# Critical-Infrastructure-Systems-Lab/ldsr

Hardware: AMD Instinct MI355X
Metric: restart x EM-iteration / s (T=1000, p=1, q=2) (higher is better)
Workload: dtype f64; 1 GPU; cfg2: synthetic T=1000 p=1 q=2, 1 series x 4096 restarts/GPU, niter=100, tol=0, dense mask; cells_rank0=4096, cells_total=4096, niter=100, algo=3

## Files before the change

### ldsr_amd/csrc/em_pair_impl.h

```cpp
#pragma once
#include "em_scan_impl.h"

__host__ __device__ constexpr long pair_image_doubles(int L, int PP, int QQ, int LPC = 32) {
    return img_doubles(L, LPC, PP, QQ);
}
__host__ __device__ constexpr long pair_strip_doubles(int L) { return (long)64 * (L - 1); }

__host__ __device__ constexpr long pair_tri_doubles(int PP, int QQ, int LPC = 32) {
    return (long)LPC * 2 * scan_pairs(PP, QQ);
}
#ifndef LDSR_STEADY
#define LDSR_STEADY 1
#endif
#ifndef LDSR_STEADY_PF
#define LDSR_STEADY_PF 4
#endif
#ifndef LDSR_STEADY_PF2
#define LDSR_STEADY_PF2 6
#endif
#ifndef LDSR_LEAD_CLOSED_VAR
#define LDSR_LEAD_CLOSED_VAR 1
#endif
#ifndef LDSR_STEADY_SBMASK
#define LDSR_STEADY_SBMASK 0x6
// ... 537 lines not shown
                    for (int p_ = 0; p_ < PP; p_++) bu = fma(th.B[p_], un[p_], bu);
                    if constexpr (LPF) {
                        const int jn = min(j + 1, nj - 1);
#pragma unroll
                        for (int p_ = 0; p_ < PP; p_++) un[p_] = lup[(long)jn * LPC * PP + p_];
                    }
                    bl = fma(A, bl, bu);
                    if constexpr (!LDSR_LEAD_CLOSED_VAR) {
                        ql = fma(A2, ql, Q);
                        al *= A;
                        a2l *= A2;
                    }
                }
            }
            if constexpr (LDSR_LEAD_CLOSED_VAR) {
                double pa = A, pa2 = A2;
#pragma unroll
                for (int bit = 0; bit < 10; bit++) {
                    if ((nj >> bit) & 1) { al *= pa; a2l *= pa2; }
                    pa *= pa; pa2 *= pa2;
                }
                const double omA2 = 1.0 - A2;
                var_closed = fabs(omA2) > 0.0009765625;
                if (var_closed) {
                    const double romA2 = fast_rcp(omA2);
                    geo = (1.0 - a2l) * romA2;
                    ql = Q * geo;
                    geo2 = ((double)nj - geo) * romA2;
                } else {
                    for (int j = 0; j < nj; j++) ql = fma(A2, ql, Q);
                }
            }
#define LSCAN_ROUND(AB, BB, A2B, QB)                                       \
            {                                                              \
                const double ab = AB, bb = BB, a2b = A2B, qb = QB;         \
                bl = fma(al, bb, bl);  al *= ab;                           \
                ql = fma(a2l, qb, ql); a2l *= a2b;                         \
            }
            LSCAN_ROUND(dpp1<DPP_ROW_SHR(1)>(al), dppz<DPP_ROW_SHR(1)>(bl), dpp1<DPP_ROW_SHR(1)>(a2l), dppz<DPP_ROW_SHR(1)>(ql))
            LSCAN_ROUND(dpp1<DPP_ROW_SHR(2)>(al), dppz<DPP_ROW_SHR(2)>(bl), dpp1<DPP_ROW_SHR(2)>(a2l), dppz<DPP_ROW_SHR(2)>(ql))
            LSCAN_ROUND(dpp1<DPP_ROW_SHR(4)>(al), dppz<DPP_ROW_SHR(4)>(bl), dpp1<DPP_ROW_SHR(4)>(a2l), dppz<DPP_ROW_SHR(4)>(ql))
            LSCAN_ROUND(dpp1<DPP_ROW_SHR(8)>(al), dppz<DPP_ROW_SHR(8)>(bl), dpp1<DPP_ROW_SHR(8)>(a2l), dppz<DPP_ROW_SHR(8)>(ql))
            if constexpr (LPC == 32)
                LSCAN_ROUND((dppd<DPP_ROW_BCAST15, 0xA>(1.0, al)), (dppd<DPP_ROW_BCAST15, 0xA>(0.0, bl)),
                            (dppd<DPP_ROW_BCAST15, 0xA>(1.0, a2l)), (dppd<DPP_ROW_BCAST15, 0xA>(0.0, ql)))
#undef LSCAN_ROUND
            double Xl = fma(al, th.mu1, bl), Vl = fma(a2l, th.V1, ql);
            x_t1 = shfl_d(Xl, hbase | (LPC - 1));
            v_t1 = shfl_d(Vl, hbase | (LPC - 1));
            Xl = dppd<DPP_WAVE_SHR1, 0xF>(th.mu1, Xl);
            Vl = dppd<DPP_WAVE_SHR1, 0xF>(th.V1, Vl);
            if (vl == 0) { Xl = th.mu1; Vl = th.V1; }
            const double rV1 = fast_rcp(v_t1);
            const double As = fabs(A) < 1e-150 ? copysign(1e-150, A) : A;
            const double rA = fast_rcp(As);
            const int k0 = lead - tA;
            const double xl2 = (double)k0 * (log_pos(fabs(As)) * 1.4426950408889634074);
            const double ef = fmin(fmax(floor(xl2), -1.0e6), 1.0e6);
            double dm = exp2(xl2 - ef);
            int de = (int)ef;
            if (As < 0.0 && (k0 & 1)) dm = -dm;
            dm *= rV1;
            de += __builtin_amdgcn_frexp_exp(dm);
            dm = __builtin_amdgcn_frexp_mant(dm);
            c_first = __builtin_amdgcn_ldexp(dm, de) * Vl;
            c_first = shfl_d(c_first, hbase);
            l_X = Xl; l_V = Vl; l_dm = dm; l_de = de; l_rA = rA; l_nj = nj;
            l_closed = var_closed; l_geo = geo; l_geo2 = geo2;
        }

        double likq = 0.0, lsp = 0.0, tLv = 0.0, X0v = 0.0, V0v = 0.0;
        int sneg = 0;
        double aSyx, aTx1x, aPall, aSxx = 0.0;
        double aSxv[QQ], aTx1u[PP], aTux[PP];
        auto zero_sums = [&]() {
            aSyx = 0.0; aTx1x = 0.0; aPall = 0.0;
#pragma unroll
            for (int q_ = 0; q_ < QQ; q_++) aSxv[q_] = 0.0;
#pragma unroll
            for (int p_ = 0; p_ < PP; p_++) { aTx1u[p_] = 0.0; aTux[p_] = 0.0; }
        };

        SCAN_TICK(0)
        if (alive) {
            PairSweepOut<PP, QQ> o;
            pair_generic_sweeps<PP, QQ, L, LPC, DENSE>(o, th, ys, hs, obsmask, lane, nl, rp, x_t1, v_t1);
            aSyx = o.aSyx; aTx1x = o.aTx1x; aPall = o.aPall; aSxx = o.aSxx;
            likq = o.likq; lsp = o.lsp; tLv = o.tLv; X0v = o.X0v; V0v = o.V0v; sneg = o.sneg;
#pragma unroll
            for (int q_ = 0; q_ < QQ; q_++) aSxv[q_] = o.aSxv[q_];
#pragma unroll
            for (int p_ = 0; p_ < PP; p_++) { aTx1u[p_] = o.aTx1u[p_]; aTux[p_] = o.aTux[p_]; }
        } else {
            zero_sums();
        }

        SCAN_TICK(6)
        if constexpr (LEAD) {
            const double dlt = shfl_d(X0v, hbase) - x_t1;
            const double *lup = lu + (long)vl * PP;
            constexpr bool LPF = LPC == 32;
            const int nj = l_nj;
            const double rA = l_rA;
            double Xl = l_X, Vl = l_V, dm = l_dm;
            int de = l_de;
#pragma unroll
            for (int i = 0; i < NLS; i++) lS[i] = 0.0;
            double c = __builtin_amdgcn_ldexp(dm, de) * Vl;
            double Xs = fma(c, dlt, Xl);
            auto lead2 = [&](int j, const double (&ul)[PP]) {
                double bu = 0.0;
#pragma unroll
                for (int p_ = 0; p_ < PP; p_++) bu = fma(th.B[p_], ul[p_], bu);
                const double Xl1 = fma(A, Xl, bu), Vl1 = fma(A2, Vl, Q);
                dm *= rA;
                if ((j & 3) == 3) { de += __builtin_amdgcn_frexp_exp(dm); dm = __builtin_amdgcn_frexp_mant(dm); }
                const double c1 = __builtin_amdgcn_ldexp(dm, de) * Vl1;
                const double Xs1 = fma(c1, dlt, Xl1);
                lS[0] = fma(Xs, Xs, lS[0]);
                if constexpr (!LDSR_LEAD_CLOSED_VAR) lS[1] += Vl;
                lS[2] = fma(c, c, lS[2]);
                lS[3] = fma(Xs1, Xs, lS[3]);
                lS[4] = fma(c, c1, lS[4]);
#pragma unroll
                for (int p_ = 0; p_ < PP; p_++) {
                    lS[5 + p_] = fma(Xs1, ul[p_], lS[5 + p_]);
                    lS[5 + PP + p_] = fma(ul[p_], Xs, lS[5 + PP + p_]);
                }
                Xl = Xl1; Vl = Vl1; c = c1; Xs = Xs1;
            };
            if constexpr (lead_pipe(PP)) {
                const int nA = (lead + LPC - 1) / LPC;
                lead_walk<PP, LPC>(lup, nj, nA, lead2);
            } else {
                double un2[PP];
#pragma unroll
                for (int p_ = 0; p_ < PP; p_++) un2[p_] = (LPF && nj > 0) ? lup[p_] : 0.0;
                for (int j = 0; j < nj; j++) {
                    double ul[PP];
                    if constexpr (!LPF) {
#pragma unroll
                        for (int p_ = 0; p_ < PP; p_++) un2[p_] = lup[(long)j * LPC * PP + p_];
                    }
#pragma unroll
                    for (int p_ = 0; p_ < PP; p_++) ul[p_] = un2[p_];
                    if constexpr (LPF) {
                        const int jn = min(j + 1, nj - 1);
#pragma unroll
                        for (int p_ = 0; p_ < PP; p_++) un2[p_] = lup[(long)jn * LPC * PP + p_];
                    }
                    lead2(j, ul);
                }
            }
            if constexpr (LDSR_LEAD_CLOSED_VAR) {
                if (l_closed) {
                    lS[1] = fma(l_V, l_geo, Q * l_geo2);
                } else {
                    double vv = l_V;
                    for (int j = 0; j < nj; j++) { lS[1] += vv; vv = fma(A2, vv, Q); }
                }
            }
        }
        SCAN_TICK(5)
        Sums<PP, QQ> S;
        {
            constexpr int NB = 5 + (DENSE ? 0 : 1);
            constexpr int NT = NB + QQ + 2 * PP;
            constexpr int NR = NT + (LEAD ? NLS : 0);
            constexpr int NSL = (NR + LPC - 1) / LPC;
            static_assert(NSL <= 4, "reduction gather: at most four slots per lane");
            double red[NR];
            if constexpr (LEAD) {
#pragma unroll
                for (int i = 0; i < NLS; i++) red[NT + i] = lS[i];
            }
            red[0] = aSyx; red[1] = aTx1x; red[2] = aPall; red[3] = likq; red[4] = lsp;
            if (!DENSE) red[5] = aSxx;
#pragma unroll
            for (int q_ = 0; q_ < QQ; q_++) red[NB + q_] = aSxv[q_];
#pragma unroll
            for (int p_ = 0; p_ < PP; p_++) { red[NB + QQ + p_] = aTx1u[p_]; red[NB + QQ + PP + p_] = aTux[p_]; }
            red_rounds<NR, LPC / 2>(red, lane);
            {
                double tt[NSL];
#pragma unroll
                for (int k_ = 0; k_ < NSL; k_++) tt[k_] = red[k_];
#pragma unroll
                for (int i = 0; i < NR; i++) red[i] = shfl_d(tt[red_slot(i, NR, LPC)], hbase | red_home(i, NR, LPC));
            }
            S.X0 = shfl_d(X0v, hbase);
            S.V0 = shfl_d(V0v, hbase);
            const double termLast = shfl_d(tLv, hbase | lastLane);
            if constexpr (LEAD) {
                const double dlt = S.X0 - x_t1, eps = S.V0 - v_t1;
                const double *l = red + NT;
                red[2] += (l[0] + l[1]) + eps * l[2];
                red[1] += l[3] + fma(eps, l[4], A * l[1]);
#pragma unroll
                for (int p_ = 0; p_ < PP; p_++) {
                    red[NB + QQ + p_] += l[5 + p_];
                    red[NB + QQ + PP + p_] += l[5 + PP + p_];
                }
                S.X0 = fma(c_first, dlt, th.mu1);
                S.V0 = fma(c_first * c_first, eps, th.V1);
            }
            const double term0 = fma(S.X0, S.X0, S.V0);
            const unsigned long long negm = __ballot(sneg < 0);
            const bool neg = ((negm >> hbase) & ((1ull << LPC) - 1ull)) != 0;
            S.Syx = red[0]; S.Tx1x = red[1];
            S.Sxx = DENSE ? red[2] : red[5];
#pragma unroll
            for (int q_ = 0; q_ < QQ; q_++) S.Sxv[q_] = red[NB + q_];
#pragma unroll
            for (int p_ = 0; p_ < PP; p_++) { S.Tx1u[p_] = red[NB + QQ + p_]; S.Tux[p_] = red[NB + QQ + PP + p_]; }
            S.Txx = red[2] - termLast;
            S.Tx1x1 = red[2] - term0;
            lik2 = lik1;
            lik1 = lik;
            lik = (-0.5 * n_obs * LDSR_LOG_2PI - 0.5 * (red[3] + red[4])) / n_obs;
            if (neg) lik = NAN;
        }
        SCAN_TICK(8)
        int abort_now = 0;
        if (prm.abort && ((++wit) & 63) == 0)
            abort_now = __builtin_amdgcn_readfirstlane(lane == 0 ? ldsr_poll_abort(prm.abort) : 0);
        if (alive && prm.liks && vl == 0) prm.liks[(long)cell * prm.niter + it] = lik;
        it++;
        bool stop = it >= prm.niter || abort_now;
        if (it >= 3 && fabs(lik - lik1) < prm.tol && fabs(lik1 - lik2) < prm.tol) stop = true;
        if (alive && stop) {
            white_out(th, (SeriesConstK)sc);
            if (vl == 0) {
                store_theta(th, prm.theta + (long)cell * P, prm.p, prm.q);
                if (prm.liks && prm.liks_nanfill)
                    for (int i = it; i < prm.niter; i++) prm.liks[(long)cell * prm.niter + i] = NAN;
                prm.n_iter[cell] = it;
                prm.lik[cell] = lik;
                prm.status[cell] = (abort_now && it < prm.niter) ? 3 : (isfinite(lik) ? 0 : 1);
#ifdef LDSR_SCAN_TIMING
                tick_[9] = __builtin_amdgcn_s_memrealtime() - real0_;
                if (prm.liks && prm.niter >= 10)
                    for (int k_ = 0; k_ < 10; k_++) prm.liks[(long)cell * prm.niter + k_] = (double)tick_[k_];
#endif
            }
            alive = false;
            if constexpr (QUEUE) {
                if (abort_now) {
                    for (int pulls = 0; pulls <= nc; pulls++) {
                        int kn = 0;
                        if (vl == 0) kn = atomicAdd(prm.queue + s, 1);
                        kn = __shfl(kn, hbase, 64);
                        if (kn >= nc) break;
                        if (vl == 0) mark_cell_interrupted(prm, c0 + kn);
                    }
                }
                if (!abort_now) {
                    int kn = 0;
                    if (vl == 0) kn = atomicAdd(prm.queue + s, 1);
                    kn = __shfl(kn, hbase, 64);
                    if (kn < nc) {
                        alive = true;
                        cell = c0 + kn;
                        load_theta(th, prm.theta0 + (long)cell * P, prm.p, prm.q, prm.has_u, prm.has_v);
                        white_in(th, (SeriesConstK)sc);
                        it = 0;
                        lik = NAN; lik1 = NAN; lik2 = NAN;
                    }
                }
            }
        } else {
            mstep_update_white<PP, QQ>(th, S, (SeriesConstK)sc, T);
        }
    }
}


struct PairEnv {
    int T, p, q, has_u, has_v, niter, liks_nanfill, n_obs;
    double tol;
    const SeriesConst *sc;
    int *queue_s;
    const int *perm;
    const double *theta0;
    double *theta, *lik, *liks;
    int *n_iter, *status;
    const int *abort;
};
template <int PP, int QQ>
struct PairCarry {
    Theta<PP, QQ> th;
    double lik, lik1, lik2;
    int it, cell, wit;
    bool alive;
#ifdef LDSR_SCAN_TIMING
    unsigned long long tick_[10], last_, real0_;
#endif
};
#ifdef LDSR_SCAN_TIMING
#define PAIR_TICK_REFS auto &tick_ = cs.tick_; auto &last_ = cs.last_;
#else
#define PAIR_TICK_REFS
#endif

__device__ __forceinline__ int pair_cell_at(const PairEnv &E, int c0, int pos) { return E.perm ? E.perm[c0 + pos] : c0 + pos; }

__device__ __forceinline__ void pair_mark_interrupted(const PairEnv &E, int cell) {
    const int P = 6 + E.p + E.q;
    for (int k = 0; k < P; k++) E.theta[(long)cell * P + k] = NAN;
    if (E.liks && E.liks_nanfill)
        for (int i = 0; i < E.niter; i++) E.liks[(long)cell * E.niter + i] = NAN;
    E.n_iter[cell] = 0;
    E.lik[cell] = NAN;
    E.status[cell] = 3;
}

struct PairVarBlk { double Vp, sg, r0, K, Vu, AVu, J, Vp1; bool st; };
template <int L>
__device__ __forceinline__ PairVarBlk pair_var_block(double V1, double A, double C, double Q, double R, bool live,
                                                     int vl, int hbase, bool shape_ok) {
    constexpr int LPC = 32, NTR = L - 1;
    PairVarBlk b;
    const double A2 = A * A, C2 = C * C;
    const double C2R = C2 * fast_rcp(R), alpha = fma(Q, C2R, A2);
    const bool trl = vl < NTR;
    double Vp;
    {
        const double mxs = fmax(alpha, 1.0);
        const int ke = -__builtin_amdgcn_frexp_exp(mxs);
        const double cs = __builtin_amdgcn_ldexp(1.0, ke);
        double p00 = trl ? alpha * cs : 1.0, p01 = trl ? Q * cs : 0.0;
        double p10 = trl ? C2R * cs : 0.0, p11 = trl ? cs : 1.0;
#define VSCAN_ROUND(Q00, Q01, Q10, Q11)                                                      \
        {                                                                            \
            const double q00 = Q00, q01 = Q01, q10 = Q10, q11 = Q11;                 \
            const double r00 = fma(p00, q00, p01 * q10), r01 = fma(p00, q01, p01 * q11); \
            const double r10 = fma(p10, q00, p11 * q10), r11 = fma(p10, q01, p11 * q11); \
            p00 = r00; p01 = r01; p10 = r10; p11 = r11;                              \
        }
#define VSCAN_SHR(n) VSCAN_ROUND(dpp1<DPP_ROW_SHR(n)>(p00), dppz<DPP_ROW_SHR(n)>(p01), dppz<DPP_ROW_SHR(n)>(p10), dpp1<DPP_ROW_SHR(n)>(p11))
        VSCAN_SHR(1) VSCAN_SHR(2) VSCAN_SHR(4)
        {
            const double m = fmax(fmax(fabs(p00), fabs(p01)), fmax(fabs(p10), fabs(p11)));
            const int e2 = 1 - __builtin_amdgcn_frexp_exp(m);
            p00 = __builtin_amdgcn_ldexp(p00, e2); p01 = __builtin_amdgcn_ldexp(p01, e2);
            p10 = __builtin_amdgcn_ldexp(p10, e2); p11 = __builtin_amdgcn_ldexp(p11, e2);
        }
        VSCAN_SHR(8)
        VSCAN_ROUND((dppd<DPP_ROW_BCAST15, 0xA>(1.0, p00)), (dppd<DPP_ROW_BCAST15, 0xA>(0.0, p01)),
                    (dppd<DPP_ROW_BCAST15, 0xA>(0.0, p10)), (dppd<DPP_ROW_BCAST15, 0xA>(1.0, p11)))
#undef VSCAN_SHR
#undef VSCAN_ROUND
        double n_e = fma(p00, V1, p01), d_e = fma(p10, V1, p11);
        n_e = dppd<DPP_WAVE_SHR1, 0xF>(V1, n_e);
        d_e = dppd<DPP_WAVE_SHR1, 0xF>(1.0, d_e);
        if (vl == 0) { n_e = V1; d_e = 1.0; }
        Vp = n_e * fast_rcp(d_e);
    }
    const double sg = fma(C2, Vp, R);
    const double r0 = fast_rcp(sg);
    const double w = Vp * r0;
    b.K = C * w;
    b.Vu = R * w;
    b.Vp1 = fma(A2, b.Vu, Q);
    b.AVu = A * b.Vu;
    b.J = b.AVu * fast_rcp(b.Vp1);
    b.Vp = Vp; b.sg = sg; b.r0 = r0;
    const double dV = b.Vp1 - Vp;
    const bool conv = fabs(dV) <= 3.552713678800501e-15 * fabs(Vp) && Vp > 0.0 && b.J * b.J < 0.8;
    const unsigned long long okm = __ballot(sg > 0.0 && sg < INFINITY);
    const unsigned long long cvm = __ballot(conv);
    constexpr unsigned long long CELL = (1ull << LPC) - 1ull;
    const unsigned long long hm = (okm >> hbase) & CELL, hc = (cvm >> hbase) & CELL;
    b.st = live && hm == CELL && ((hc >> (LPC - 1)) & 1ull) != 0ull && shape_ok;
    return b;
}

template <int PP, int QQ, bool QUEUE>
__device__ __forceinline__ void pair_steady_finish(const PairEnv &E, PairCarry<PP, QQ> &cs, const PairSweepOut<PP, QQ> &o,
                                                   double addTx1x, double addPall, bool active, int lane, int c0,
                                                   int nc, int lastLane) {
    constexpr int LPC = 32;
    PAIR_TICK_REFS
    const int vl = lane & 31, hbase = lane & 32;
    const int P = 6 + E.p + E.q;
    Sums<PP, QQ> S;
    {
        constexpr int NB = 5;
        constexpr int NR = NB + QQ + 2 * PP;
        double red[NR];
        red[0] = o.aSyx; red[1] = o.aTx1x; red[2] = o.aPall; red[3] = o.likq; red[4] = o.lsp;
#pragma unroll
        for (int q_ = 0; q_ < QQ; q_++) red[NB + q_] = o.aSxv[q_];
#pragma unroll
        for (int p_ = 0; p_ < PP; p_++) { red[NB + QQ + p_] = o.aTx1u[p_]; red[NB + QQ + PP + p_] = o.aTux[p_]; }
        red_rounds<NR, LPC / 2>(red, lane);
        {
            const double tt = red[0];
#pragma unroll
            for (int i = 0; i < NR; i++) red[i] = shfl_d(tt, hbase | red_home(i, NR, LPC));
        }
        S.X0 = shfl_d(o.X0v, hbase);
        S.V0 = shfl_d(o.V0v, hbase);
        const double termLast = shfl_d(o.tLv, hbase | lastLane);
        red[1] += addTx1x; red[2] += addPall;
        const double term0 = fma(S.X0, S.X0, S.V0);
        const unsigned long long negm = __ballot(o.sneg < 0);
        const bool neg = ((negm >> hbase) & ((1ull << LPC) - 1ull)) != 0;
        S.Syx = red[0]; S.Tx1x = red[1];
        S.Sxx = red[2];
#pragma unroll
        for (int q_ = 0; q_ < QQ; q_++) S.Sxv[q_] = red[NB + q_];
#pragma unroll
        for (int p_ = 0; p_ < PP; p_++) { S.Tx1u[p_] = red[NB + QQ + p_]; S.Tux[p_] = red[NB + QQ + PP + p_]; }
        S.Txx = red[2] - termLast;
        S.Tx1x1 = red[2] - term0;
        if (active) {
            cs.lik2 = cs.lik1;
            cs.lik1 = cs.lik;
            cs.lik = (-0.5 * E.n_obs * LDSR_LOG_2PI - 0.5 * (red[3] + red[4])) / E.n_obs;
            if (neg) cs.lik = NAN;
        }
    }
    SCAN_TICK(8)
    int abort_now = 0;
    if (E.abort && ((++cs.wit) & 63) == 0)
        abort_now = __builtin_amdgcn_readfirstlane(lane == 0 ? ldsr_poll_abort(E.abort) : 0);
    if (active && E.liks && vl == 0) E.liks[(long)cs.cell * E.niter + cs.it] = cs.lik;
    if (active) cs.it++;
    bool stop = active && cs.it >= E.niter;
    if (active && cs.it >= 3 && fabs(cs.lik - cs.lik1) < E.tol && fabs(cs.lik1 - cs.lik2) < E.tol) stop = true;
    if (cs.alive && abort_now) stop = true;
    if (cs.alive && stop) {
        white_out(cs.th, (SeriesConstK)E.sc);
        if (vl == 0) {
            store_theta(cs.th, E.theta + (long)cs.cell * P, E.p, E.q);
            if (E.liks && E.liks_nanfill)
                for (int i = cs.it; i < E.niter; i++) E.liks[(long)cs.cell * E.niter + i] = NAN;
            E.n_iter[cs.cell] = cs.it;
            E.lik[cs.cell] = cs.lik;
            E.status[cs.cell] = (abort_now && cs.it < E.niter) ? 3 : (isfinite(cs.lik) ? 0 : 1);
#ifdef LDSR_SCAN_TIMING
            tick_[9] = __builtin_amdgcn_s_memrealtime() - cs.real0_;
            if (E.liks && E.niter >= 10)
                for (int k_ = 0; k_ < 10; k_++) E.liks[(long)cs.cell * E.niter + k_] = (double)tick_[k_];
#endif
        }
        cs.alive = false;
        if constexpr (QUEUE) {
            if (abort_now) {
                for (int pulls = 0; pulls <= nc; pulls++) {
                    int kn = 0;
                    if (vl == 0) kn = atomicAdd(E.queue_s, 1);
                    kn = __shfl(kn, hbase, 64);
                    if (kn >= nc) break;
                    if (vl == 0) pair_mark_interrupted(E, pair_cell_at(E, c0, kn));
                }
            } else {
                int kn = 0;
                if (vl == 0) kn = atomicAdd(E.queue_s, 1);
                kn = __shfl(kn, hbase, 64);
                if (kn < nc) {
                    cs.alive = true;
                    cs.cell = pair_cell_at(E, c0, kn);
                    load_theta(cs.th, E.theta0 + (long)cs.cell * P, E.p, E.q, E.has_u, E.has_v);
                    white_in(cs.th, (SeriesConstK)E.sc);
                    cs.it = 0;
                    cs.lik = NAN; cs.lik1 = NAN; cs.lik2 = NAN;
                }
            }
        }
    } else if (active) {
        mstep_update_white<PP, QQ>(cs.th, S, (SeriesConstK)E.sc, E.T);
    }
}

template <int PP, int QQ, int L, bool QUEUE>
__device__ __attribute__((noinline)) PairCarry<PP, QQ> pair_steady_g_phase(PairEnv Ev, PairCarry<PP, QQ> cs, bool slow,
                                                                           int c0, int nc) {
    constexpr int LPC = 32;
    extern __shared__ __attribute__((aligned(16))) double smem[];
    PAIR_TICK_REFS
    auto ui = [](int x) { return __builtin_amdgcn_readfirstlane(x); };
    auto up = [&](auto *ptr) {
        const unsigned long long v = (unsigned long long)ptr;
        const unsigned lo = (unsigned)__builtin_amdgcn_readfirstlane((int)(unsigned)v);
        const unsigned hi = (unsigned)__builtin_amdgcn_readfirstlane((int)(unsigned)(v >> 32));
        return (decltype(ptr))(((unsigned long long)hi << 32) | lo);
    };
    PairEnv E;
    E.T = ui(Ev.T); E.p = ui(Ev.p); E.q = ui(Ev.q); E.has_u = ui(Ev.has_u); E.has_v = ui(Ev.has_v);
    E.niter = ui(Ev.niter); E.liks_nanfill = ui(Ev.liks_nanfill); E.n_obs = ui(Ev.n_obs);
    E.tol = uniform_d(Ev.tol);
    E.sc = up(Ev.sc); E.queue_s = up(Ev.queue_s); E.perm = up(Ev.perm); E.theta0 = up(Ev.theta0);
    E.theta = up(Ev.theta); E.lik = up(Ev.lik); E.liks = up(Ev.liks); E.n_iter = up(Ev.n_iter);
    E.status = up(Ev.status); E.abort = up(Ev.abort);
    c0 = ui(c0); nc = ui(nc);
    const int lane = threadIdx.x & 63, wave = threadIdx.x >> 6;
    const int vl = lane & 31, hbase = lane & 32;
    const int T = E.T;
    const int nl = (T + L - 1) / L, rp = T - nl * (L - 1);
    const bool shape_ok = rp >= 1 && nl > 1;
    const double *ys = smem;
    double *hs = smem + pair_image_doubles(L, PP, QQ, LPC) + (long)wave * pair_strip_doubles(L) + lane;
    do {
        SCAN_TICK(7)
        PairSweepOut<PP, QQ> o;
        pair_generic_sweeps<PP, QQ, L, LPC, true>(o, cs.th, ys, hs, 0u, lane, nl, rp, cs.th.mu1, cs.th.V1);
        SCAN_TICK(6)
        pair_steady_finish<PP, QQ, QUEUE>(E, cs, o, 0.0, 0.0, slow, lane, c0, nc, nl - 1);
        const PairVarBlk vb = pair_var_block<L>(cs.th.V1, cs.th.A, cs.th.C, cs.th.Q, cs.th.R, cs.alive, vl, hbase, shape_ok);
        slow = cs.alive && !vb.st;
    } while (__any(slow));
    return cs;
}

template <int PP, int QQ, int L, bool QUEUE>
__device__ __forceinline__ void em_pair_body_steady(const EmParams &prm, const double *ys, double *hs,
                                                    const double *tri, int s, int c0, int nc, int lane,
                                                    int wave) {
    constexpr int LPC = 32;
    constexpr int KP = scan_pairs(PP, QQ), KV = img_values(PP, QQ);
    constexpr int NTR = L - 1;
    static_assert(NTR < LPC, "the last lane of the cell is the template, not a transient step");
    const int vl = lane & 31, hbase = lane & 32;
    auto val = [&](int j, int i) -> double { return ys[img_off(j, i, KV, LPC, L) + vl * 2]; };
    auto ldw = [&](int j, double (&w)[2 * KP]) {
#pragma unroll
        for (int i = 0; i < KV; i++) w[i] = val(j, i);
    };
    constexpr int PF = KP <= 2 ? LDSR_STEADY_PF : (KP <= 4 ? 2 : 1);
    constexpr int PF2 = LDSR_STEADY_PF2;
    const int T = prm.T;
    const int P = 6 + prm.p + prm.q;
    PairEnv E;
    E.T = T; E.p = prm.p; E.q = prm.q; E.has_u = prm.has_u; E.has_v = prm.has_v;
    E.niter = prm.niter; E.liks_nanfill = prm.liks_nanfill; E.tol = prm.tol;
    E.sc = prm.sc + s; E.n_obs = E.sc->n_obs;
    E.queue_s = prm.queue + s; E.perm = prm.perm; E.theta0 = prm.theta0;
    E.theta = prm.theta; E.lik = prm.lik; E.liks = prm.liks; E.n_iter = prm.n_iter; E.status = prm.status;
    E.abort = prm.abort;
    const int nl = (T + L - 1) / L;
    const int rp = T - nl * (L - 1);
    const bool act = vl < nl;
    const bool tail = vl < rp;
    const int lastLane = nl - 1;
    const bool shape_ok = rp >= 1 && nl > 1;

    PairCarry<PP, QQ> cs;
    int k = QUEUE ? 0 : 2 * wave + (lane >> 5);
    if constexpr (QUEUE) {
        if (vl == 0) k = atomicAdd(E.queue_s, 1);
        k = __shfl(k, hbase, 64);
    }
    cs.alive = k < nc;
    cs.cell = pair_cell_at(E, c0, cs.alive ? k : 0);
    load_theta(cs.th, prm.theta0 + (long)cs.cell * P, prm.p, prm.q, prm.has_u, prm.has_v);
    white_in(cs.th, (SeriesConstK)E.sc);
    cs.lik = NAN; cs.lik1 = NAN; cs.lik2 = NAN;
    cs.it = 0;
    cs.wit = 0;
#ifdef LDSR_SCAN_TIMING
    for (int k_ = 0; k_ < 10; k_++) cs.tick_[k_] = 0;
    cs.last_ = __builtin_readcyclecounter();
    cs.real0_ = __builtin_amdgcn_s_memrealtime();
#endif
    PAIR_TICK_REFS
    Theta<PP, QQ> &th = cs.th;

    while (__any(cs.alive)) {
        bool slow = false;
        while (__any(cs.alive)) {
            SCAN_TICK(7)
            const double A = th.A, C = th.C;
            const PairVarBlk vb = pair_var_block<L>(th.V1, A, C, th.Q, th.R, cs.alive, vl, hbase, shape_ok);
            const bool st = vb.st;
            slow = cs.alive && !st;
            if (__builtin_expect(__any(slow), 0)) break;
            double likq = 0.0, lsp = 0.0, tLv = 0.0, X0v = 0.0, V0v = 0.0;
            double addPall = 0.0, addTx1x = 0.0;
            double aSyx = 0.0, aTx1x = 0.0, aPall = 0.0;
            double aSxv[QQ], aTx1u[PP], aTux[PP];
            auto zero_sums = [&]() {
                aSyx = 0.0; aTx1x = 0.0; aPall = 0.0;
#pragma unroll
                for (int q_ = 0; q_ < QQ; q_++) aSxv[q_] = 0.0;
#pragma unroll
                for (int p_ = 0; p_ < PP; p_++) { aTx1u[p_] = 0.0; aTux[p_] = 0.0; }
            };
            const bool trl = vl < NTR;
            auto tval = [&](int i) -> double { return tri[((i >> 1) * LPC + vl) * 2 + (i & 1)]; };
            double e_t = tval(0), bu_t = 0.0;
#pragma unroll
            for (int q_ = 0; q_ < QQ; q_++) e_t = fma(-th.D[q_], tval(1 + PP + q_), e_t);
#pragma unroll
            for (int p_ = 0; p_ < PP; p_++) bu_t = fma(th.B[p_], tval(1 + p_), bu_t);
            const double K = vb.K, J = vb.J, Vu = vb.Vu, AVu = vb.AVu, r0 = vb.r0;
            double Xp;
            {
                const double aKt = A * K;
                double al = trl ? fma(-aKt, C, A) : 1.0, bl = trl ? fma(aKt, e_t, bu_t) : 0.0;
#define MSCAN_ROUND(AB, BB) { const double ab = AB, bb = BB; bl = fma(al, bb, bl); al *= ab; }
                MSCAN_ROUND(dpp1<DPP_ROW_SHR(1)>(al), dppz<DPP_ROW_SHR(1)>(bl))
                MSCAN_ROUND(dpp1<DPP_ROW_SHR(2)>(al), dppz<DPP_ROW_SHR(2)>(bl))
                MSCAN_ROUND(dpp1<DPP_ROW_SHR(4)>(al), dppz<DPP_ROW_SHR(4)>(bl))
                MSCAN_ROUND(dpp1<DPP_ROW_SHR(8)>(al), dppz<DPP_ROW_SHR(8)>(bl))
                MSCAN_ROUND((dppd<DPP_ROW_BCAST15, 0xA>(1.0, al)), (dppd<DPP_ROW_BCAST15, 0xA>(0.0, bl)))
#undef MSCAN_ROUND
                Xp = fma(al, th.mu1, bl);
                Xp = dppd<DPP_WAVE_SHR1, 0xF>(th.mu1, Xp);
                if (vl == 0) Xp = th.mu1;
            }
            const double dl = fma(-C, Xp, e_t);
            const double Xu = fma(K, dl, Xp);
            const double Xp1 = fma(A, Xu, bu_t);
            const double trJ = J;
            const double trG = fma(-J, Xp1, Xu);
            const double trH = fma(-J, AVu, Vu);
            const double trLq = trl ? dl * r0 * dl : 0.0;
            const double lg = log_pos(vb.sg);
            const double trLg = trl ? lg : 0.0;
            const int src = hbase | (LPC - 1);
            const double cK = shfl_d(K, src), cJ = shfl_d(J, src), cr = shfl_d(r0, src), cVu = shfl_d(Vu, src);
            const double ch = shfl_d(trH, src), clg = shfl_d(lg, src), X_tr = shfl_d(Xp, src);

            SCAN_TICK(0)
            if (st) {
                const bool body = act && vl >= 1;
                const bool tail_s = tail;
                const double aK = A * cK, a = fma(-aK, C, A);
                double aL = 1.0, JL = 1.0;
                {
                    double sa = a, sj = cJ;
                    bool have = false;
#pragma unroll
                    for (int bit = 0; (1 << bit) <= L - 1; bit++) {
                        if ((L - 1) & (1 << bit)) {
                            if (!have) { aL = sa; JL = sj; have = true; }
                            else { aL *= sa; JL *= sj; }
                        }
                        if ((2 << bit) <= L - 1) { sa *= sa; sj *= sj; }
                    }
                }
                double gv_[L];
                double al = 1.0, bl = 0.0, buLast = 0.0;
                auto f1s = [&](int j, const double (&w)[2 * KP]) {
                    double e = w[0], bu = 0.0;
#pragma unroll
                    for (int q_ = 0; q_ < QQ; q_++) e = fma(-th.D[q_], w[1 + PP + q_], e);
#pragma unroll
                    for (int p_ = 0; p_ < PP; p_++) bu = fma(th.B[p_], w[1 + p_], bu);
                    gv_[j] = e;
                    if (j < L - 1) hs[j * 64] = bu; else buLast = bu;
                    bl = fma(a, bl, fma(aK, e, bu));
                };
                {
                    constexpr bool PRET = KP <= 4;
                    double Wt[2 * KP], W[PF][2 * KP];
                    if constexpr (PRET) ldw(L - 1, Wt);
#pragma unroll
                    for (int d = 0; d < PF; d++) ldw(d, W[d]);
                    __builtin_amdgcn_sched_barrier(LDSR_STEADY_SBMASK);
                    if (body) {
#pragma unroll
                        for (int j = 0; j < L - 1; j++) {
                            f1s(j, W[j % PF]);
                            if (j + PF < L - 1) ldw(j + PF, W[j % PF]);
                            __builtin_amdgcn_sched_barrier(LDSR_STEADY_SBMASK);
                        }
                        al = aL;
                    }
                    if (tail_s) {
                        if constexpr (!PRET) ldw(L - 1, Wt);
                        f1s(L - 1, Wt);
                        al *= a;
                    }
                }
#define SSCAN_ROUND(AB, BB) { const double ab = AB, bb = BB; bl = fma(al, bb, bl); al *= ab; }
                SSCAN_ROUND(dpp1<DPP_ROW_SHR(1)>(al), dppz<DPP_ROW_SHR(1)>(bl))
                SSCAN_ROUND(dpp1<DPP_ROW_SHR(2)>(al), dppz<DPP_ROW_SHR(2)>(bl))
                SSCAN_ROUND(dpp1<DPP_ROW_SHR(4)>(al), dppz<DPP_ROW_SHR(4)>(bl))
                SSCAN_ROUND(dpp1<DPP_ROW_SHR(8)>(al), dppz<DPP_ROW_SHR(8)>(bl))
                SSCAN_ROUND((dppd<DPP_ROW_BCAST15, 0xA>(1.0, al)), (dppd<DPP_ROW_BCAST15, 0xA>(0.0, bl)))
#undef SSCAN_ROUND
                SCAN_TICK(1)
                double Xq = fma(al, X_tr, bl);
                Xq = dppd<DPP_WAVE_SHR1, 0xF>(X_tr, Xq);
                if (vl == 0) Xq = X_tr;
                double lq = 0.0, Xuq = 0.0;
                auto f2s = [&](int j, double bu) {
                    const double e = gv_[j];
                    const double dlq = fma(-C, Xq, e);
                    lq = fma(dlq, dlq, lq);
                    Xuq = fma(cK, dlq, Xq);
                    const double Xq1 = fma(A, Xuq, bu);
                    double g = fma(-cJ, Xq1, Xuq);
                    if (j >= L - 2) {
                        const bool fin = (vl == lastLane) && (j == (tail_s ? L - 1 : L - 2));
                        g = fin ? Xuq : g;
                    }
                    gv_[j] = g;
                    Xq = Xq1;
                };
                if (body) {
                    double U[PF2];
#pragma unroll
                    for (int d = 0; d < PF2; d++) U[d] = hs[d * 64];
                    __builtin_amdgcn_sched_barrier(LDSR_STEADY_SBMASK);
#pragma unroll
                    for (int j = 0; j < L - 1; j++) {
                        f2s(j, U[j % PF2]);
                        if (j + PF2 < L - 1) U[j % PF2] = hs[(j + PF2) * 64];
                        __builtin_amdgcn_sched_barrier(LDSR_STEADY_SBMASK);
                    }
                }
                if (tail_s) f2s(L - 1, buLast);
                SCAN_TICK(2)
                constexpr bool PRET2 = KP <= 4;
                double Vt[2 * KP], V[PF][2 * KP];
                if constexpr (PRET2) {
                    ldw(L - 1, Vt);
#pragma unroll
                    for (int d = 0; d < PF; d++) ldw(L - 2 - d, V[d]);
                }
                __builtin_amdgcn_sched_barrier(LDSR_STEADY_SBMASK);
                tLv = fma(Xuq, Xuq, cVu);
                const int nst = (body ? L - 1 : 0) + (tail_s ? 1 : 0);
                likq = fma(cr, lq, trLq);
                lsp = fma((double)nst, clg, trLg);
                double Pi = 1.0, G = 0.0;
                if (tail_s) { G = gv_[L - 1]; Pi = cJ; }
                if (body) {
#pragma unroll
                    for (int j = L - 2; j >= 0; j--) G = fma(cJ, G, gv_[j]);
                    Pi *= JL;
                }
#define RSCAN_ROUND(n) { const double Pb = dpp1<DPP_ROW_SHL(n)>(Pi), Gb = dppz<DPP_ROW_SHL(n)>(G); G = fma(Pi, Gb, G); Pi *= Pb; }
                RSCAN_ROUND(1) RSCAN_ROUND(2) RSCAN_ROUND(4) RSCAN_ROUND(8)
#undef RSCAN_ROUND
                {
                    double Hdummy = 0.0;
                    rscan_cross<LPC>(Pi, G, Hdummy, lane);
                }
                double Xn = dppd<DPP_WAVE_SHL1, 0xF>(0.0, G);
                if (vl == LPC - 1) Xn = 0.0;
                const double XsS = shfl_d(G, hbase);
                SCAN_TICK(3)
                zero_sums();
                auto b2s = [&](int j, const double (&w)[2 * KP]) {
                    const double Xs = fma(cJ, Xn, gv_[j]);
                    aTx1x = fma(Xn, Xs, aTx1x);
#pragma unroll
                    for (int p_ = 0; p_ < PP; p_++) {
                        const double ut = w[1 + p_];
                        aTx1u[p_] = fma(Xn, ut, aTx1u[p_]);
                        aTux[p_] = fma(ut, Xs, aTux[p_]);
                    }
                    aPall = fma(Xs, Xs, aPall);
                    aSyx = fma(w[0], Xs, aSyx);
#pragma unroll
                    for (int q_ = 0; q_ < QQ; q_++) aSxv[q_] = fma(Xs, w[1 + PP + q_], aSxv[q_]);
                    Xn = Xs;
                };
                if constexpr (!PRET2) {
                    if (tail_s) ldw(L - 1, Vt);
#pragma unroll
                    for (int d = 0; d < PF; d++) ldw(L - 2 - d, V[d]);
                }
                if (tail_s) b2s(L - 1, Vt);
                if (body) {
#pragma unroll
                    for (int j = L - 2; j >= 0; j--) {
                        const int d = (L - 2 - j) % PF;
                        b2s(j, V[d]);
                        if (j - PF >= 0) ldw(j - PF, V[d]);
                        __builtin_amdgcn_sched_barrier(LDSR_STEADY_SBMASK);
                    }
                }
                SCAN_TICK(4)
                const int N = T - NTR;
                const double rho = cJ * cJ;
                const double romr = fast_rcp(1.0 - rho);
                const double Vss = ch * romr;
                const double dV = cVu - Vss;
                const double VsS = Vss;
                const double sumVs = fma(dV, romr, (double)N * Vss);
                addPall = sumVs;
                addTx1x = cJ * (sumVs - VsS);
                {
                    int vl2 = vl;
                    asm volatile("" : "+v"(vl2));
                    auto tval2 = [&](int i) -> double { return tri[((i >> 1) * LPC + vl2) * 2 + (i & 1)]; };
                    double Pt = trl ? trJ : 1.0, Gt = trl ? trG : 0.0, Ht = trl ? trH : 0.0;
#define RSCAN_ROUND(n)                                                     \
                    {                                                          \
                        const double Pb = dpp1<DPP_ROW_SHL(n)>(Pt);            \
                        const double Gb = dppz<DPP_ROW_SHL(n)>(Gt);            \
                        const double Hb = dppz<DPP_ROW_SHL(n)>(Ht);            \
                        Gt = fma(Pt, Gb, Gt);                                  \
                        Ht = fma(Pt * Pt, Hb, Ht);                             \
                        Pt *= Pb;                                              \
                    }
                    RSCAN_ROUND(1) RSCAN_ROUND(2) RSCAN_ROUND(4) RSCAN_ROUND(8)
#undef RSCAN_ROUND
                    rscan_cross<LPC>(Pt, Gt, Ht, lane);
                    const double XsT = fma(Pt, XsS, Gt), VsT = fma(Pt * Pt, VsS, Ht);
                    const double XsN = dppd<DPP_WAVE_SHL1, 0xF>(0.0, XsT);
                    const double VsN = dppd<DPP_WAVE_SHL1, 0xF>(0.0, VsT);
                    if (trl) {
                        aTx1x = fma(XsN, XsT, fma(VsN, trJ, aTx1x));
#pragma unroll
                        for (int p_ = 0; p_ < PP; p_++) {
                            const double ut = tval2(1 + p_);
                            aTx1u[p_] = fma(XsN, ut, aTx1u[p_]);
                            aTux[p_] = fma(ut, XsT, aTux[p_]);
                        }
                        aPall += fma(XsT, XsT, VsT);
                        aSyx = fma(tval2(0), XsT, aSyx);
#pragma unroll
                        for (int q_ = 0; q_ < QQ; q_++) aSxv[q_] = fma(XsT, tval2(1 + PP + q_), aSxv[q_]);
                    }
                    X0v = XsT; V0v = VsT;
                }
            } else {
                zero_sums();
            }
            SCAN_TICK(5)
            PairSweepOut<PP, QQ> o;
            o.aSyx = aSyx; o.aTx1x = aTx1x; o.aPall = aPall; o.aSxx = 0.0;
            o.likq = likq; o.lsp = lsp; o.tLv = tLv; o.X0v = X0v; o.V0v = V0v; o.sneg = 0;
#pragma unroll
            for (int q_ = 0; q_ < QQ; q_++) o.aSxv[q_] = aSxv[q_];
#pragma unroll
            for (int p_ = 0; p_ < PP; p_++) { o.aTx1u[p_] = aTx1u[p_]; o.aTux[p_] = aTux[p_]; }
            pair_steady_finish<PP, QQ, QUEUE>(E, cs, o, addTx1x, addPall, st, lane, c0, nc, lastLane);
        }
        if (__builtin_expect(!__any(slow), 1)) break;
        cs = pair_steady_g_phase<PP, QQ, L, QUEUE>(E, cs, slow, c0, nc);
    }
}

template <int PP, int QQ, int L, int LPC, bool QUEUE, bool LEAD = false>
__global__ __launch_bounds__(512) void em_pair_kernel(EmParams prm) {
    extern __shared__ __attribute__((aligned(16))) double smem[];
    constexpr long IMG = pair_image_doubles(L, PP, QQ, LPC);
    const int b = blockIdx.x;
    const int s = prm.blk_series[b];
    const int c0 = prm.blk_cell0[b], nc = prm.blk_ncell[b];
    const int lane = threadIdx.x & 63, wave = threadIdx.x >> 6;
    const double *gimg = prm.img2 + (long)s * prm.img2_stride;
    for (int i = threadIdx.x; i < (int)IMG; i += blockDim.x) smem[i] = gimg[i];
    constexpr long STRIP = pair_strip_doubles(L);
    double *lu = smem + IMG + (long)(blockDim.x >> 6) * STRIP;
    if constexpr (LEAD) {
        const int n3 = ((prm.lead + LPC - 1) / LPC) * LPC * PP;
        const double *g3 = prm.img3 + (long)s * prm.img3_stride;
        for (int i = threadIdx.x; i < n3; i += blockDim.x) lu[i] = g3[i];
    }
    constexpr bool STEADY = !LEAD && pair_steady(L, LPC, PP, QQ);
    const double *tri = lu;
    if constexpr (STEADY) {
        constexpr int KP = scan_pairs(PP, QQ);
        constexpr int NTR = pair_steady_ntr(L, LPC);
        for (int i = threadIdx.x; i < KP * LPC * 2; i += blockDim.x) {
            const int c = i & 1, l = (i >> 1) % LPC, m = (i >> 1) / LPC;
            const int vi = 2 * m + c;
            lu[i] = (l < NTR && vi < img_values(PP, QQ)) ? gimg[img_off(l % L, vi, img_values(PP, QQ), LPC, L) + (l / L) * 2] : 0.0;
        }
    }
    __syncthreads();
    const SeriesConst *sc = prm.sc + s;
    if (sc->status != 0) {
        const int P = 6 + prm.p + prm.q;
        for (int c = threadIdx.x; c < nc; c += blockDim.x) {
            const int cell = c0 + c;
            for (int k = 0; k < P; k++) prm.theta[(long)cell * P + k] = NAN;
            prm.n_iter[cell] = 0;
            if (prm.liks && prm.liks_nanfill)
                for (int i = 0; i < prm.niter; i++) prm.liks[(long)cell * prm.niter + i] = NAN;
            prm.lik[cell] = NAN;
            prm.status[cell] = 2;
        }
        return;
    }
    if (!QUEUE && (64 / LPC) * wave >= nc) return;
    double *hs = smem + IMG + (long)wave * STRIP + lane;
    const bool dense = sc->n_obs == prm.T;
    if constexpr (LEAD) {
        em_pair_body<PP, QQ, L, LPC, false, QUEUE, true>(prm, smem, hs, lu, s, c0, nc, lane, wave);
    } else {
        if (dense) {
            if constexpr (STEADY) em_pair_body_steady<PP, QQ, L, QUEUE>(prm, smem, hs, tri, s, c0, nc, lane, wave);
            else em_pair_body<PP, QQ, L, LPC, true, QUEUE, false>(prm, smem, hs, lu, s, c0, nc, lane, wave);
        } else {
            em_pair_body<PP, QQ, L, LPC, false, QUEUE, false>(prm, smem, hs, lu, s, c0, nc, lane, wave);
        }
    }
}

struct PairPlan {
    int L = 0;
    int lpc = 0;
    int wpb = 0;
    bool ok = false;
};
PairPlan pair_plan(int T, int PP, int QQ, int lpc, bool lead_form = false);

template <int L, int LPC>
hipError_t launch_em_pair_L(const EmParams &prm, int PPv, int QQv, int n_blocks, int wpb, bool queue,
                            hipStream_t stream);
__host__ __device__ constexpr long pair_lead_doubles(int lead, int LPC, int PP) {
    return (long)((lead + LPC - 1) / LPC) * LPC * PP;
}
```

Baseline: 567.6 million restart*EM-iter/s.

## Replace variance Möbius scan with closed-form Riccati solution and pass carry via LDS

The per-lane predicted-variance recursion was computed with a wave-level DPP prefix scan of 2x2 matrix products. It now uses the closed-form solution of the scalar Riccati recurrence: it takes the eigenvalues of the Möbius map, forms rho, and raises it to the lane's step with five squarings. This removes the cross-lane DPP rounds and rescaling. Separately, the noinline slow-path function now receives and returns the carry state through the wave's LDS strip instead of by value, which is meant to cut call-boundary register pressure in the hot steady loop. The risks are numerical differences near alpha≈1, where the two eigenvalues nearly coincide, and extra LDS traffic when the slow path is taken.

Measured after the change: 572.4 million restart*EM-iter/s, median of 6. About the same (+0.8%).

```diff
diff --git a/ldsr_amd/csrc/em_pair_impl.h b/ldsr_amd/csrc/em_pair_impl.h
--- a/ldsr_amd/csrc/em_pair_impl.h
+++ b/ldsr_amd/csrc/em_pair_impl.h
@@ -863,6 +863,44 @@
 #define PAIR_TICK_REFS
 #endif
 
+template <int PP, int QQ>
+__host__ __device__ constexpr int pair_carry_slots() {
+#ifdef LDSR_SCAN_TIMING
+    return 6 + PP + QQ + 5 + 12;
+#else
+    return 6 + PP + QQ + 5;
+#endif
+}
+template <int PP, int QQ, typename D, typename I>
+__device__ __forceinline__ void pair_carry_fields(PairCarry<PP, QQ> &cs, D &&dbl, I &&two_ints, int &alive) {
+    dbl(cs.th.A); dbl(cs.th.C); dbl(cs.th.Q); dbl(cs.th.R); dbl(cs.th.mu1); dbl(cs.th.V1);
+#pragma unroll
+    for (int p_ = 0; p_ < PP; p_++) dbl(cs.th.B[p_]);
+#pragma unroll
+    for (int q_ = 0; q_ < QQ; q_++) dbl(cs.th.D[q_]);
+    dbl(cs.lik); dbl(cs.lik1); dbl(cs.lik2);
+    two_ints(cs.it, cs.cell);
+    two_ints(cs.wit, alive);
+#ifdef LDSR_SCAN_TIMING
+#pragma unroll
+    for (int k_ = 0; k_ < 10; k_++) dbl(cs.tick_[k_]);
+    dbl(cs.last_); dbl(cs.real0_);
+#endif
+}
+template <int PP, int QQ>
+__device__ __forceinline__ void pair_carry_store(double *hs, PairCarry<PP, QQ> &cs) {
+    int k = 0, alive = cs.alive;
+    pair_carry_fields(cs, [&](auto &x) { *reinterpret_cast<std::remove_reference_t<decltype(x)> *>(hs + 64 * k++) = x; },
+                      [&](int &a, int &b) { int *w = reinterpret_cast<int *>(hs + 64 * k++); w[0] = a; w[1] = b; }, alive);
+}
+template <int PP, int QQ>
+__device__ __forceinline__ void pair_carry_load(const double *hs, PairCarry<PP, QQ> &cs) {
+    int k = 0, alive = 0;
+    pair_carry_fields(cs, [&](auto &x) { x = *reinterpret_cast<const std::remove_reference_t<decltype(x)> *>(hs + 64 * k++); },
+                      [&](int &a, int &b) { const int *w = reinterpret_cast<const int *>(hs + 64 * k++); a = w[0]; b = w[1]; }, alive);
+    cs.alive = alive != 0;
+}
+
 __device__ __forceinline__ int pair_cell_at(const PairEnv &E, int c0, int pos) { return E.perm ? E.perm[c0 + pos] : c0 + pos; }
 
 __device__ __forceinline__ void pair_mark_interrupted(const PairEnv &E, int cell) {
@@ -880,40 +918,31 @@
 __device__ __forceinline__ PairVarBlk pair_var_block(double V1, double A, double C, double Q, double R, bool live,
                                                      int vl, int hbase, bool shape_ok) {
     constexpr int LPC = 32, NTR = L - 1;
+    static_assert(NTR < 32, "rho^t takes five squarings");
     PairVarBlk b;
     const double A2 = A * A, C2 = C * C;
     const double C2R = C2 * fast_rcp(R), alpha = fma(Q, C2R, A2);
     const bool trl = vl < NTR;
     double Vp;
     {
-        const double mxs = fmax(alpha, 1.0);
-        const int ke = -__builtin_amdgcn_frexp_exp(mxs);
-        const double cs = __builtin_amdgcn_ldexp(1.0, ke);
-        double p00 = trl ? alpha * cs : 1.0, p01 = trl ? Q * cs : 0.0;
-        double p10 = trl ? C2R * cs : 0.0, p11 = trl ? cs : 1.0;
-#define VSCAN_ROUND(Q00, Q01, Q10, Q11)                                                      \
-        {                                                                            \
-            const double q00 = Q00, q01 = Q01, q10 = Q10, q11 = Q11;                 \
-            const double r00 = fma(p00, q00, p01 * q10), r01 = fma(p00, q01, p01 * q11); \
-            const double r10 = fma(p10, q00, p11 * q10), r11 = fma(p10, q01, p11 * q11); \
-            p00 = r00; p01 = r01; p10 = r10; p11 = r11;                              \
-        }
-#define VSCAN_SHR(n) VSCAN_ROUND(dpp1<DPP_ROW_SHR(n)>(p00), dppz<DPP_ROW_SHR(n)>(p01), dppz<DPP_ROW_SHR(n)>(p10), dpp1<DPP_ROW_SHR(n)>(p11))
-        VSCAN_SHR(1) VSCAN_SHR(2) VSCAN_SHR(4)
-        {
-            const double m = fmax(fmax(fabs(p00), fabs(p01)), fmax(fabs(p10), fabs(p11)));
-            const int e2 = 1 - __builtin_amdgcn_frexp_exp(m);
-            p00 = __builtin_amdgcn_ldexp(p00, e2); p01 = __builtin_amdgcn_ldexp(p01, e2);
-            p10 = __builtin_amdgcn_ldexp(p10, e2); p11 = __builtin_amdgcn_ldexp(p11, e2);
-        }
-        VSCAN_SHR(8)
-        VSCAN_ROUND((dppd<DPP_ROW_BCAST15, 0xA>(1.0, p00)), (dppd<DPP_ROW_BCAST15, 0xA>(0.0, p01)),
-                    (dppd<DPP_ROW_BCAST15, 0xA>(0.0, p10)), (dppd<DPP_ROW_BCAST15, 0xA>(1.0, p11)))
-#undef VSCAN_SHR
-#undef VSCAN_ROUND
-        double n_e = fma(p00, V1, p01), d_e = fma(p10, V1, p11);
-        n_e = dppd<DPP_WAVE_SHR1, 0xF>(V1, n_e);
-        d_e = dppd<DPP_WAVE_SHR1, 0xF>(1.0, d_e);
+        const double am1 = alpha - 1.0, cQ = C2R * Q;
+        const double sd = sqrt(fma(am1, am1, 4.0 * cQ));
+        const double big = 0.5 * (sd + fabs(am1));
+        const double sml = cQ * fast_rcp(big);
+        const bool up = am1 >= 0.0;
+        const double Pe = up ? big : sml, Ne = up ? sml : big;
+        const double rl = fast_rcp(1.0 + Pe);
+        const double rho = (A2 * rl) * rl;
+        const int t = trl ? vl : NTR;
+        double rt = 1.0, sq = rho;
+#pragma unroll
+        for (int bit = 0; bit < 5; bit++) {
+            rt = (t & (1 << bit)) ? rt * sq : rt;
+            if (bit < 4) sq = sq * sq;
+        }
+        const double omr = 1.0 - rt;
+        double n_e = fma(V1, fma(rt, Ne, Pe), Q * omr);
+        double d_e = fma(C2R * V1, omr, fma(rt, Pe, Ne));
         if (vl == 0) { n_e = V1; d_e = 1.0; }
         Vp = n_e * fast_rcp(d_e);
     }
@@ -1036,11 +1065,10 @@
 }
 
 template <int PP, int QQ, int L, bool QUEUE>
-__device__ __attribute__((noinline)) PairCarry<PP, QQ> pair_steady_g_phase(PairEnv Ev, PairCarry<PP, QQ> cs, bool slow,
-                                                                           int c0, int nc) {
+__device__ __attribute__((noinline)) void pair_steady_g_phase(PairEnv Ev, bool slow, int c0, int nc) {
     constexpr int LPC = 32;
+    static_assert(pair_carry_slots<PP, QQ>() <= L - 1, "the carry fits the lane's strip");
     extern __shared__ __attribute__((aligned(16))) double smem[];
-    PAIR_TICK_REFS
     auto ui = [](int x) { return __builtin_amdgcn_readfirstlane(x); };
     auto up = [&](auto *ptr) {
         const unsigned long long v = (unsigned long long)ptr;
@@ -1063,6 +1091,9 @@
     const bool shape_ok = rp >= 1 && nl > 1;
     const double *ys = smem;
     double *hs = smem + pair_image_doubles(L, PP, QQ, LPC) + (long)wave * pair_strip_doubles(L) + lane;
+    PairCarry<PP, QQ> cs;
+    pair_carry_load(hs, cs);
+    PAIR_TICK_REFS
     do {
         SCAN_TICK(7)
         PairSweepOut<PP, QQ> o;
@@ -1072,7 +1103,7 @@
         const PairVarBlk vb = pair_var_block<L>(cs.th.V1, cs.th.A, cs.th.C, cs.th.Q, cs.th.R, cs.alive, vl, hbase, shape_ok);
         slow = cs.alive && !vb.st;
     } while (__any(slow));
-    return cs;
+    pair_carry_store(hs, cs);
 }
 
 template <int PP, int QQ, int L, bool QUEUE>
@@ -1396,7 +1427,9 @@
             pair_steady_finish<PP, QQ, QUEUE>(E, cs, o, addTx1x, addPall, st, lane, c0, nc, lastLane);
         }
         if (__builtin_expect(!__any(slow), 1)) break;
-        cs = pair_steady_g_phase<PP, QQ, L, QUEUE>(E, cs, slow, c0, nc);
+        pair_carry_store(hs, cs);
+        pair_steady_g_phase<PP, QQ, L, QUEUE>(E, slow, c0, nc);
+        pair_carry_load(hs, cs);
     }
 }
 
```
